# JeremyCCHsu/vae-npvc

Measured on AMD Instinct MI355X. Metric: SP frames/sec (train step: fwd+bwd+Adam), higher is better.
Workload: dtype f32 tensors and accumulation / bf16x2 operands (16 mantissa bits) on the matrix cores

## Files before the change

vae-npvc_amd/csrc/gfx950_fbwd.h:

```cpp
#pragma once
#include "gfx950_fwgrad.h"

namespace vaenpvc {
namespace tuned {

enum { FB_D2, FB_D1, FB_E1, FB_COUNT };
constexpr int FB_DY2_PITCH = 516;
constexpr bool fb_enc(int l) { return l == FB_E1; }
constexpr int fb_gsite(int l) { return l == FB_D2 ? CV_D2G : l == FB_D1 ? CV_D1G : CV_E1G; }
constexpr int fb_wsite(int l) { return l == FB_D2 ? CW_D2 : l == FB_D1 ? CW_D1 : CW_E1; }
constexpr int fb_cgr(int l) { return l == FB_D2 ? 1 : l == FB_D1 ? 2 : 4; }
#ifndef VAENPVC_FB_PFW
#define VAENPVC_FB_PFW 0x330
#endif
constexpr int fb_pfw(int l) { return (VAENPVC_FB_PFW >> (4 * l)) & 0xf; }

#ifndef VAENPVC_FB_OTL
#define VAENPVC_FB_OTL 1
#endif
#ifndef VAENPVC_FB_ABL
#define VAENPVC_FB_ABL 0
#endif
#ifndef VAENPVC_FB_XROT
#define VAENPVC_FB_XROT 0x313
// ... 7 lines not shown
  static constexpr CvSite V = CVS[fb_gsite(L)];
  static constexpr CwSite WS = CWS[fb_wsite(L)];
  static constexpr ClDesc GD = CLD[ENC ? WS.a : WS.b], XD = CLD[ENC ? WS.b : WS.a];
  static constexpr int CG = GD.C, HG = GD.H, NG = CG * HG, CX = XD.C, HX = XD.H;
  static constexpr int R = WS.R, R16 = rup(R, 16), TAPS = WS.T, S = 3;
  static constexpr int CPLG = (CG == 32 || CG == 64 || CG == 128) ? CG + 8 : CG;
  static constexpr int CPLX = (CX == 32 || CX == 64 || CX == 128) ? CX + 8 : CX;
  static constexpr int VIEWROWS = S * (R16 - 1) + TAPS + 1;
  static constexpr int ROW0G = GD.HLO, ROWSG = ENC ? fb_max(GD.HP, GD.HLO + R16) : VIEWROWS;
  static constexpr int ROW0X = ENC ? XD.HLO : 0, ROWSX = ENC ? VIEWROWS : R16;
  static constexpr int GPL = ROWSG * CPLG + 64, XPL = ROWSX * CPLX + 64;
  static constexpr int KS = cdiv(V.NT * CG, 16), MT = cdiv(V.M, 32), WP = V.Kp + 8, WPL = MT * 32 * WP;
  static constexpr int RSTEP = (V.step / CG) * CPLG;
  static constexpr int CVW = ENC ? CX : CG, CPLV = ENC ? CPLX : CPLG, CPN = ENC ? CG : CX, CPLN = ENC ? CPLG : CPLX;
  static constexpr int N = TAPS * CVW, M = WS.M, NT = cdiv(N, 32), MTW = cdiv(M, 32);
  static constexpr int KSPLIT = NT <= 2 ? 2 : 1, WN = 4 / KSPLIT, NTW = cdiv(NT, WN);
  static constexpr int CGR = fb_cgr(L), CUG = CG / CGR, NCHG = cdiv(HG, 64), NITG = NCHG * CGR, IPWG = cdiv(NITG, 4);
  static constexpr bool OTL = VAENPVC_FB_OTL != 0;
  static constexpr bool LNB2_OK = OTL && L == FB_D1 && NPL <= 2;
  static constexpr ClDesc PD0 = CLD[CL_GD0];
  static constexpr int P0_CPL = PD0.CP + 8, P0_IMG = PD0.HP * P0_CPL;
  static constexpr int OFR = CX * HX, LDS_IMG = NPL * (GPL + XPL + WPL) * 2, LDS = LDS_IMG + (OTL ? OFR * 4 : 0);
  static constexpr int LDS_LNB2 = LDS + OFR * 4 + 2 * NPL * P0_IMG * 2;
  static_assert(!OTL || (LDS_IMG % 16 == 0 && OFR % 4 == 0), "result tile: aligned, whole pieces");
  static_assert(V.x == (ENC ? WS.a : WS.b) && GD.CP == CG && XD.CP == CX && M == CPN && CUG == 8 && 4 % CGR == 0, "layer not served");
  static_assert(V.OC == CX && V.OH == HX && V.PH == (ENC ? 1 : 0) && (ENC || (V.R == R && MT == 1)), "layer not served");
  static_assert(KS * 16 <= V.Kp && (V.R - 1) * RSTEP + (KS * 16 / CG + 1) * CPLG <= ROWSG * CPLG + 64, "view runs past the frame image");
};

struct FbArgs {
  const float* dy;
  const float* a;
  const float* st;
  const float* gamma;
  const float* beta;
  const float* xa;
  const float* xst;
  const float* xgamma;
  const float* xbeta;
  const unsigned short* W;
  float* dx;
  float* dW;
  float* dgamma;
  float* dbeta;
  float* dbias;
  int F;
  bool bf16_act = false;
  int dy_pitch = 0;
  unsigned short* pl0 = nullptr;
  int64_t pl0_plane = 0;
  float* part0 = nullptr;
};

#ifndef VAENPVC_FB_OCC3
#define VAENPVC_FB_OCC3 0
#endif
#ifndef VAENPVC_FB_MAXPL
#define VAENPVC_FB_MAXPL 3
#endif
constexpr int fb_occ(int l, bool lnb2) { return (!lnb2 && ((VAENPVC_FB_OCC3 >> l) & 1)) ? 3 : 2; }
template <int NPL, int L, int BFM = 0, int DYP = 0, bool LNB2 = false>
__global__ void __launch_bounds__(256, fb_occ(L, LNB2)) k_fbwd(FbArgs a) {
  using T = FbCfg<NPL, L>;
  static_assert(!LNB2 || (T::LNB2_OK && BFM == 0), "LayerNorm backward of the layer below: decoder layer 1, fp32 storage");
  constexpr bool BFG = BFM & 1, BFX = (BFM >> 1) & 1, BFO = (BFM >> 2) & 1;
  constexpr int PG = act_pitch(BFG, T::HG), PO = act_pitch(BFO, T::V.OH), PD = DYP ? DYP : PG;
  static_assert(DYP == 0 || (BFM == 0 && DYP >= T::HG), "padded rows: fp32 storage");
  static_assert(BFM == 0 || (NPL == 1 && !T::ENC), "bf16 storage: decoder layers of the bf16 mode");
  constexpr CvSite V = T::V;
  constexpr int CUG = T::CUG, HG = T::HG, CGR = T::CGR, NITG = T::NITG, IPWG = T::IPWG;
  extern __shared__ __attribute__((aligned(16))) unsigned short bsm[];
  __shared__ float part[2][FbCfg<NPL, L>::NITG];
  __shared__ float red[4][3 * FbCfg<NPL, L>::CUG];
  __shared__ float lnx[2][FbCfg<NPL, L>::CX];
  __shared__ float red0[2][4][2];
  __shared__ float lnq0[2][LNB2 ? FbCfg<NPL, L>::CX : 1];
  float* xh0 = reinterpret_cast<float*>(reinterpret_cast<unsigned char*>(bsm) + T::LDS);
  unsigned short* img0 = reinterpret_cast<unsigned short*>(xh0 + T::OFR);
  unsigned short* gs = bsm;
  unsigned short* xs = bsm + NPL * T::GPL;
  unsigned short* ws = xs + NPL * T::XPL;
  const int tid = threadIdx.x, lane = tid & 63, wave = __builtin_amdgcn_readfirstlane(tid >> 6), l31 = lane & 31, lh = lane >> 5;
  const int cg = wave % CGR;
  const int xwave = (wave + T::XROT) & 3;
  float gam[CUG], bet[CUG];
#pragma unroll
  for (int c = 0; c < CUG; ++c) {
    gam[c] = __builtin_bit_cast(float, __builtin_amdgcn_readfirstlane(__builtin_bit_cast(int, a.gamma[cg * CUG + c])));
    bet[c] = __builtin_bit_cast(float, __builtin_amdgcn_readfirstlane(__builtin_bit_cast(int, a.beta[cg * CUG + c])));
  }
  float vd[IPWG][CUG], va[IPWG][CUG], mean = 0.f, rstd = 1.f;
  FwStage<NPL, T::CX, T::CX, T::CPLX, T::HX, 1, 0, T::ROW0X, T::XPL, BFX> sx;
  float su[CUG], sw[CUG], sd[CUG];
#pragma unroll
  for (int c = 0; c < CUG; ++c) su[c] = sw[c] = sd[c] = 0.f;

  auto uload = [&](int f, auto which_) __attribute__((always_inline)) {
    constexpr int WHICH = decltype(which_)::value;
    if constexpr ((WHICH & 2) != 0) {
      mean = a.st[2 * f];
      rstd = a.st[2 * f + 1];
// ... 84 lines not shown
    const u32x4 z = {0u, 0u, 0u, 0u};
    for (int i = tid; i < NPL * (T::GPL + T::XPL) / 8; i += 256) reinterpret_cast<u32x4*>(bsm)[i] = z;
    constexpr int WROW8 = V.Kp / 8, WPIECES = NPL * T::MT * 32 * WROW8;
    for (int i = tid; i < WPIECES; i += 256) {
      const int p = i / (T::MT * 32 * WROW8), r = i - p * (T::MT * 32 * WROW8), m = r / WROW8, c8 = r - m * WROW8;
      *reinterpret_cast<u32x4*>(ws + p * T::WPL + m * T::WP + c8 * 8) =
          *reinterpret_cast<const u32x4*>(a.W + ((size_t)p * V.Mp + m) * V.Kp + c8 * 8);
    }
  }
  const int c0 = tid >> 3, t8 = tid & 7;
  float g0 = 0.f, b0 = 0.f, su0 = 0.f, sw0 = 0.f, sd0 = 0.f;
  if constexpr (LNB2) {
    g0 = a.xgamma[c0];
    b0 = a.xbeta[c0];
    const u32x4 z = {0u, 0u, 0u, 0u};
    for (int i = tid; i < 2 * NPL * T::P0_IMG / 8; i += 256) reinterpret_cast<u32x4*>(img0)[i] = z;
    if (blockIdx.x == 0) {
      const int64_t used = (int64_t)a.F * T::PD0.HP * T::PD0.CP;
      for (int64_t i = used + tid; i < a.pl0_plane; i += 256)
#pragma unroll
        for (int p = 0; p < NPL; ++p) a.pl0[p * a.pl0_plane + i] = 0;
    }
  }
  auto copy_out0 = [&](int fp, int par) __attribute__((always_inline)) {
    constexpr int G8 = T::PD0.CP / 8, PPP = T::PD0.HP * G8;
    const unsigned short* im = img0 + par * NPL * T::P0_IMG;
    unsigned short* df = a.pl0 + (int64_t)fp * T::PD0.HP * T::PD0.CP;
#pragma unroll
    for (int r = 0; r < cdiv(NPL * PPP, 256); ++r) {
      const int it = min(tid + 256 * r, NPL * PPP - 1);
      const int p = it / PPP, q = it - p * PPP, hp = q / G8, g8 = q - hp * G8;
      const u32x4 v = *reinterpret_cast<const u32x4*>(im + p * T::P0_IMG + hp * T::P0_CPL + 8 * g8);
      *reinterpret_cast<u32x4*>(df + p * a.pl0_plane + (int64_t)q * 8) = v;
    }
  };
  int nfr = 0;
  int fprev = -1;
  __syncthreads();
  const int wn = wave % T::WN, kpar = wave / T::WN;
  f32x16 wacc[T::NTW][T::MTW];
#pragma unroll
  for (int i = 0; i < T::NTW; ++i)
#pragma unroll
    for (int j = 0; j < T::MTW; ++j) wacc[i][j] = zero16();
  const int trow = ((lane & 15) >> 2) + 8 * lh, tcol = 4 * (lane & 3) + 16 * ((lane >> 4) & 1);
  int vcol[T::NTW], pcol[T::MTW];
#pragma unroll
  for (int i = 0; i < T::NTW; ++i) {
    int n = 32 * (wn + i * T::WN) + tcol;
    n = n < T::N ? n : 0;
    vcol[i] = (n / T::CVW) * T::CPLV + n % T::CVW;
  }
#pragma unroll
  for (int j = 0; j < T::MTW; ++j) {
    const int m = 32 * j + tcol;
    pcol[j] = m < T::CPN ? m : 0;
  }
  const unsigned short* vimg = T::ENC ? xs : gs;
  const unsigned short* pimg = T::ENC ? gs + T::ROW0G * T::CPLG : xs;
  constexpr int VPL = T::ENC ? T::XPL : T::GPL, PPL = T::ENC ? T::GPL : T::XPL;
  const int woff = l31 * T::WP + lh * 8;
  for (; f < a.F; f += gridDim.x) {
    if (T::PFW != 3) {
      if constexpr (T::PFW != 3) uload(f, WTOP{});
      sx.load(a.xa, a.xst, f, a.F, xwave, lane);
    }
    upass1();
    sx.store(xs, true, lnx[0], lnx[1], xwave, lane, LNB2 ? xh0 : nullptr);
    __syncthreads();
    upass2();
    __syncthreads();
    if (T::PFW && f + (int)gridDim.x < a.F) {
      uload(f + gridDim.x, WPF{});
      if (T::PFW == 3) sx.load(a.xa, a.xst, f + gridDim.x, a.F, xwave, lane);
    }
    constexpr int NSTEPS = cdiv(V.R, 32);
    for (int s = (T::KSPLIT > 1 ? 3 - wave : wave); s < ((VAENPVC_FB_ABL & 1) ? 0 : NSTEPS); s += 4) {
      int q = s * 32 + l31;
      const bool nok = q < V.R;
      q = nok ? q : 0;
      const int xoff = q * T::RSTEP;
      f32x16 acc[T::MT];
#pragma unroll
      for (int i = 0; i < T::MT; ++i) acc[i] = zero16();
#pragma unroll
      for (int ks = 0; ks < T::KS; ++ks) {
        u32x4 fa[T::MT][NPL], fb[NPL];
        const int ko = fc_koff<T::CG, T::CPLG>(ks, lh);
#pragma unroll
        for (int p = 0; p < NPL; ++p) {
#pragma unroll
          for (int i = 0; i < T::MT; ++i) fa[i][p] = *reinterpret_cast<const u32x4*>(ws + p * T::WPL + i * 32 * T::WP + woff + ks * 16);
          fb[p] = *reinterpret_cast<const u32x4*>(gs + p * T::GPL + xoff + ko);
        }
        using PR = Prod<NPL>;
#pragma unroll
        for (int t = 0; t < PR::N; ++t)
// ... 105 lines not shown
        red0[par][wave][1] = s2;
      }
      __syncthreads();
      constexpr float INVN0 = 1.0f / T::OFR;
      s1 = ((red0[par][0][0] + red0[par][1][0]) + (red0[par][2][0] + red0[par][3][0])) * INVN0;
      s2 = ((red0[par][0][1] + red0[par][1][1]) + (red0[par][2][1] + red0[par][3][1])) * INVN0;
      if (fprev >= 0) copy_out0(fprev, par ^ 1);
      unsigned short* im = img0 + par * NPL * T::P0_IMG;
#pragma unroll
      for (int j = 0; j < EPT0; ++j) {
        const int h = t8 + 8 * j;
        if (h >= HX) continue;
        const float d = rstd0 * (dn[j] * g0 - s1 - xh[j] * s2);
        su0 += dn[j] * xh[j];
        sw0 += dn[j];
        sd0 += d;
        unsigned t[NPL];
        split_n<NPL>(d, t);
#pragma unroll
        for (int p = 0; p < NPL; ++p) im[p * T::P0_IMG + (T::PD0.HLO + h) * T::P0_CPL + c0] = (unsigned short)t[p];
      }
      fprev = f;
      ++nfr;
    } else if constexpr (T::OTL && BFM == 0) {
      if (!((VAENPVC_FB_ABL & (1 | 4)) && a.F > 0)) {
        const f32x4* ot4 = reinterpret_cast<const f32x4*>(reinterpret_cast<const unsigned char*>(bsm) + T::LDS_IMG);
        f32x4* og = reinterpret_cast<f32x4*>(a.dx + (int64_t)f * T::OFR);
        constexpr int N4 = T::OFR / 4;
#pragma unroll
        for (int r = 0; r < cdiv(N4, 256); ++r) {
          const int i = min(tid + 256 * r, N4 - 1);
          og[i] = ot4[i];
        }
      }
    }
  }
  if constexpr (LNB2) {
    __syncthreads();
    if (fprev >= 0) copy_out0(fprev, (nfr - 1) & 1);
#pragma unroll
    for (int o = 1; o < 8; o <<= 1) {
      su0 += __shfl_xor(su0, o);
      sw0 += __shfl_xor(sw0, o);
      sd0 += __shfl_xor(sd0, o);
    }
    if (t8 == 0) {
      float* pp = a.part0 + (int64_t)blockIdx.x * (3 * T::CX);
      pp[c0] = su0;
      pp[T::CX + c0] = sw0;
      pp[2 * T::CX + c0] = sd0;
    }
  }
  if ((VAENPVC_FB_ABL & 16) && a.F > 0) return;
#pragma unroll
  for (int i = 0; i < T::NTW; ++i)
#pragma unroll
    for (int j = 0; j < T::MTW; ++j) {
      const int m = 32 * j + l31;
      if (m >= T::M) continue;
#pragma unroll
      for (int reg = 0; reg < 16; ++reg) {
        const int n = 32 * (wn + i * T::WN) + acc_row(reg, lane);
        if (n < T::N && wn + i * T::WN < T::NT) atomicAdd(a.dW + n * T::M + m, wacc[i][j][reg]);
      }
    }
#pragma unroll
  for (int c = 0; c < CUG; ++c) {
    const float u = wave_sum(su[c]), w = wave_sum(sw[c]), d = wave_sum(sd[c]);
    if (lane == 0) {
      red[wave][c] = u;
      red[wave][CUG + c] = w;
      red[wave][2 * CUG + c] = d;
    }
  }
  __syncthreads();
  if (tid < 3 * T::CG) {
    const int which = tid / T::CG, c = tid - which * T::CG, cgi = c / CUG, cc = c - cgi * CUG;
    float v = 0.f;
#pragma unroll
    for (int w4 = 0; w4 < 4; ++w4)
      if (w4 % CGR == cgi) v += red[w4][which * CUG + cc];
    float* dst = which == 0 ? a.dgamma + c : which == 1 ? a.dbeta + c : a.dbias + c;
    atomicAdd(dst, v);
  }
}

template <int NPL, int L>
static unsigned fbwd_grid(int64_t F) {
  using T = FbCfg<NPL, L>;
  return (unsigned)cmin_((int)F, T::LDS > 78 * 1024 ? 256 : (fb_occ(L, false) == 3 && 3 * T::LDS <= 156 * 1024) ? 768 : 512);
}
static unsigned fbwd_grid_d1(int npl, int64_t F) { return npl == 1 ? fbwd_grid<1, FB_D1>(F) : fbwd_grid<2, FB_D1>(F); }

template <int NPL, int L>
static void launch_fbwd(const FbArgs& a, hipStream_t s) {
  using T = FbCfg<NPL, L>;
  const unsigned grid = fbwd_grid<NPL, L>(a.F);
  if constexpr (NPL == 1 && (L == FB_D2 || L == FB_D1)) {
    if (a.bf16_act) {
      constexpr int BFM = L == FB_D2 ? 7 : 1;
      rt().ensure_lds(reinterpret_cast<const void*>(&k_fbwd<NPL, L, BFM>), T::LDS);
      hipLaunchKernelGGL((k_fbwd<NPL, L, BFM>), dim3(grid), dim3(256), T::LDS, s, a);
      return;
    }
  }
  if constexpr (T::LNB2_OK) {
    if (a.pl0) {
      rt().ensure_lds(reinterpret_cast<const void*>(&k_fbwd<NPL, L, 0, 0, true>), T::LDS_LNB2);
      hipLaunchKernelGGL((k_fbwd<NPL, L, 0, 0, true>), dim3(grid), dim3(256), T::LDS_LNB2, s, a);
      return;
    }
  }
  if constexpr (L == FB_D2) {
    if (a.dy_pitch == FB_DY2_PITCH) {
      rt().ensure_lds(reinterpret_cast<const void*>(&k_fbwd<NPL, L, 0, FB_DY2_PITCH>), T::LDS);
      hipLaunchKernelGGL((k_fbwd<NPL, L, 0, FB_DY2_PITCH>), dim3(grid), dim3(256), T::LDS, s, a);
      return;
    }
  }
  rt().ensure_lds(reinterpret_cast<const void*>(&k_fbwd<NPL, L>), T::LDS);
  hipLaunchKernelGGL((k_fbwd<NPL, L>), dim3(grid), dim3(256), T::LDS, s, a);
}
template <int NPL>
static bool fbwd(int layer, const FbArgs& a, hipStream_t s) {
  if constexpr (NPL <= VAENPVC_FB_MAXPL) {
    switch (layer) {
      case FB_D2: launch_fbwd<NPL, FB_D2>(a, s); return true;
      case FB_D1: launch_fbwd<NPL, FB_D1>(a, s); return true;
      case FB_E1: launch_fbwd<NPL, FB_E1>(a, s); return true;
    }
  }
  return false;
}

}
// ... 2 lines not shown
```

vae-npvc_amd/csrc/gfx950_layers.hip:

```cpp
#include <cstdlib>
#include <cstring>
#include <type_traits>

#include "gfx950_convgemm.h"
#include "gfx950_convwgrad.h"
#include "gfx950_dense.h"
#include "gfx950_elem.h"
#include "gfx950_tngemm.h"
#include "gfx950_toeplitz.h"
#include "gfx950_toep_bf16.h"
#include "gfx950_planegemm.h"
#include "gfx950_ntring.h"
#include "gfx950_viewconv.h"
#include "gfx950_fconv.h"
#include "gfx950_fwgrad.h"
#include "gfx950_fconv_r.h"
#include "gfx950_fbwd.h"
#include "gfx950_lnb_planes.h"
#include "kernels.h"

namespace vaenpvc {
namespace tuned {

#ifndef E1F_T
// ... 120 lines not shown
  static constexpr int gd2 = d2f + D2F::BTOTAL;
  static constexpr int gd0 = gd2 + GD2::BTOTAL;
  static constexpr int ge4 = gd0 + GD0::BTOTAL;
  static constexpr int ge3 = ge4 + GE4::BTOTAL;
  static constexpr int ge2 = ge3 + GE3::BTOTAL;
  static constexpr int ge1 = ge2 + GE2::BTOTAL;
  static constexpr int wc = ge1 + GE1::BTOTAL;
  static constexpr int lnpart = wc + TOEP_C * WROW;
  static constexpr int wdg = lnpart + 2048 * 3 * 256;
  static constexpr int wfw = wdg + TB_WFLOATS;
  static constexpr int heads_bias = wfw + TB_WFLOATS;
  static constexpr int pg_headsf = heads_bias + 256;
  static constexpr int pg_headsb = pg_headsf + 3 * 256 * 768 / 2;
  static constexpr int pg_mergef = pg_headsb + 3 * 768 * 256 / 2;
  static constexpr int pg_mergeb = pg_mergef + 3 * 1664 * 128 / 2;
  static constexpr int pg_enc4f = pg_mergeb + 3 * 128 * 1600 / 2;
  static constexpr int pg_enc4b = pg_enc4f + 3 * 768 * 896 / 2;
  static constexpr int pg_bias4 = pg_enc4b + 3 * 896 * 768 / 2;
  static constexpr int cvw = pg_bias4 + 768;
  static constexpr int cvwr_d0f = cvw + CV_WTOTAL;
  static constexpr int cvwr_e2g = cvwr_d0f + fcr_wfloats(CV_D0F);
  static constexpr int enc0part_ = cvwr_e2g + fcr_wfloats(CV_E2G);
  static constexpr int enc0part = enc0part_;
  static constexpr int total = enc0part + 512 * 7 * 16;
};
static_assert(Pk::total <= 8 * 939162 + 65536, "packed weights must fit the scratch region");
static inline bool sel(unsigned mask, int bit) { return (mask >> bit) & 1u; }
static inline bool fwd_on(int bit) { return sel(rt().fwd_mask, bit); }
static inline bool bwd_on(int bit) { return sel(rt().bwd_mask, bit); }
constexpr unsigned SEL_STEPS = (2u << VAENPVC_SEL_DEC3) - 1;
constexpr int64_t PLANEGEMM_MIN_FRAMES = 1024;
static inline bool pg_on(unsigned mask, int64_t F) {
  return sel(mask, VAENPVC_SEL_PLANE_GEMM) && (F >= PLANEGEMM_MIN_FRAMES || !sel(mask, VAENPVC_SEL_PLANE_GEMM_MIN_FRAMES));
}
static inline bool pg_fwd(int64_t F) { return pg_on(rt().fwd_mask, F); }
static inline bool cg_fwd(int64_t F) { return fwd_on(VAENPVC_SEL_VIEW_GEMM) && pg_on(rt().fwd_mask | (1u << VAENPVC_SEL_PLANE_GEMM), F); }
static inline bool cg_bwd(int64_t F) { return bwd_on(VAENPVC_SEL_VIEW_GEMM) && pg_on(rt().bwd_mask | (1u << VAENPVC_SEL_PLANE_GEMM), F); }
static inline bool pg_bwd(int64_t F) { return pg_on(rt().bwd_mask, F); }
static inline bool pg_step(int bit, int64_t F) { return bwd_on(bit) && pg_bwd(F) && pg_fwd(F) && fwd_on(bit); }
static inline bool cv_sel(unsigned mask, int site) { return !sel(mask, VAENPVC_SEL_CV_SITE_SET) || ((rt().cv_sites() >> site) & 1u); }
static inline bool cv_fwd(int site, int64_t F) { return cg_fwd(F) && cv_sel(rt().fwd_mask, site); }
static inline bool cv_bwd(int site, int64_t F) { return cg_bwd(F) && cv_sel(rt().bwd_mask, site); }
constexpr int64_t FCONV_MIN_FRAMES = 1024;
constexpr int64_t ENC0_WAVE_MIN_FRAMES = 1024;
static inline bool enc0_wave(unsigned mask, int64_t F) { return F >= ENC0_WAVE_MIN_FRAMES || !sel(mask, VAENPVC_SEL_ENC0_WAVE_MIN_FRAMES); }
static inline bool fc_on(unsigned mask, int site, int64_t F) {
  if (!fconv_serves(site, rt().planes)) return false;
// ... 646 lines not shown
  else if (toep_planes)
    for_planes([&](auto npl) {
      constexpr int NPL_ = decltype(npl)::value;
      auto launch_dp = [&](auto kern) {
        VAENPVC_TIMED("dxh_post", s, hipLaunchKernelGGL(kern, dim3((unsigned)cmin_(2048, cdiv((int)F, 4))), dim3(256), 0, s, w.d_xh, P + m.dec[3].w_off,
                           reinterpret_cast<unsigned short*>(w.toep_gp), w.dy_tmp, G + m.dec[3].b_off, (int)F, dy2_pitch(F)));
      };
      if constexpr (NPL_ == 1) {
        if (abf) { launch_dp(k_dxh_post<1, true>); return; }
      }
      launch_dp(k_dxh_post<NPL_, false>);
    });
  ready();
  bool dec_bias_done[4] = {false, false, false, false};
  bool enc_bias_done[5] = {false, false, false, false, false};
  const int WGS = 512;
  const int LWGS = 2048;
  LnReduceList lnq_store;
  lnq_store.n = 0;
  lnq_store.used = 0;
  lnq_store.capacity = (int64_t)2048 * 3 * 256;
  LnReduceList* lnq = (F <= 512 && (rt().bwd_mask & SEL_STEPS) == SEL_STEPS) ? &lnq_store : nullptr;
  const bool enc0_fused = bwd_on(VAENPVC_SEL_ENC0) && bwd_on(VAENPVC_SEL_ENC1) && bwd_on(VAENPVC_SEL_ENC0_FUSED_BWD) && F >= ENC0_WAVE_MIN_FRAMES && !lnq;

  auto gsplit = [&](int cl, const float* src, const char* tag) {
    for_planes([&](auto npl) {
      VAENPVC_TIMED(tag, s, cv_split<decltype(npl)::value>(cl, src, nullptr, nullptr, nullptr, w.cl[cl], F, s));
    });
  };
  auto asplit = [&](int cl, const float* src, const float* st, const ConvL* ln, const char* tag) {
    for_planes([&](auto npl) {
      VAENPVC_TIMED(tag, s, cv_split<decltype(npl)::value>(cl, src, st, ln ? P + ln->gamma_off : nullptr, ln ? P + ln->beta_off : nullptr,
                                                           w.cl[cl], F, s));
    });
  };
  auto vwgrad = [&](int wsite, float* dW, const char* tag) {
    for_planes([&](auto npl) {
      VAENPVC_TIMED(tag, s2, cv_wgrad<decltype(npl)::value>(wsite, w.cl[CWS[wsite].a], w.cl[CWS[wsite].b], dW, F, 512, s2));
    });
  };
  auto fdgrad = [&](int site, const float* grad, float* out, const char* tag) {
    for_planes([&](auto npl) {
      FcArgs fa{grad, nullptr, nullptr, nullptr, nullptr, reinterpret_cast<const unsigned short*>(w.scratch + Pk::cvw + cv_woff(site)), nullptr, out, F};
      VAENPVC_TIMED(tag, s, fconv<decltype(npl)::value>(site, fa, s));
    });
  };
// ... 84 lines not shown
                                                            w.dy_tmp, (int)F, ToepLna{}));
        };
        if constexpr (NPL == 1) {
          if (abf) { launch_dg(&k_toep_gemm_bf16<false, 1, true>); return; }
        }
        if (dy2_pitch(F) == DY2_PITCH) launch_dg(&k_toep_gemm_bf16<false, NPL, false, DY2_PITCH>);
        else launch_dg(&k_toep_gemm_bf16<false, NPL, false>);
      });
    } else
    if (F >= 8192) {
      VAENPVC_TIMED("dec3_dgrad", s, hipLaunchKernelGGL((k_toep_dgrad<8, 8>), dim3((unsigned)cdiv(F, 32), 1), dim3(512), TD_LDS, s, w.d_xh,
                                                        w.scratch + Pk::wc, w.dy_tmp, F));
    } else {
      VAENPVC_TIMED("dec3_dgrad", s, hipLaunchKernelGGL((k_toep_dgrad<1, 4>), dim3((unsigned)cdiv(F, 32), 8), dim3(256), TD_LDS, s, w.d_xh,
                                                        w.scratch + Pk::wc, w.dy_tmp, F));
    }
    if (!(bwd_on(VAENPVC_SEL_DEC2) && fb_bwd(FB_D2, F))) {
      VAENPVC_TIMED("lnb_dec2", s, launch_ln_bwd<LnbCfg<8, 513>>(w.dy_tmp, w.dec_a[2], w.dec_st[2], P + l2.gamma_off, P + l2.beta_off, w.d_dec_a[2],
                                       G + l2.gamma_off, G + l2.beta_off, G + l2.b_off, w.scratch + Pk::lnpart, F, LWGS, s, lnq));
      dec_bias_done[2] = true;
    }
  } else generic::bwd_dec_layer(m, P, F, w, G, s, 3);
  auto fused_bwd = [&](int layer, int i, const float* dy, float* dx, const char* tag, unsigned short* pl0 = nullptr, int64_t pl0_plane = 0,
                       float* part0 = nullptr) {
    const bool enc = fb_enc(layer);
    const ConvL &l = enc ? m.enc[i] : m.dec[i], &pl = enc ? m.enc[i - 1] : m.dec[i - 1];
    float* const* act = enc ? w.enc_a : w.dec_a;
    float* const* sts = enc ? w.enc_st : w.dec_st;
    for_planes([&](auto npl) {
      constexpr int NPL = decltype(npl)::value;
      FbArgs fa{dy, act[i], sts[i], P + l.gamma_off, P + l.beta_off, act[i - 1], sts[i - 1], P + pl.gamma_off,
                P + pl.beta_off, reinterpret_cast<const unsigned short*>(w.scratch + Pk::cvw + cv_woff(fb_gsite(layer))), dx,
                G + l.w_off, G + l.gamma_off, G + l.beta_off, G + l.b_off, F};
      fa.bf16_act = abf && !enc;
      fa.dy_pitch = (layer == FB_D2 && dy2_pitch(F) == DY2_PITCH) ? DY2_PITCH : 0;
      fa.pl0 = pl0;
      fa.pl0_plane = pl0_plane;
      fa.part0 = part0;
      VAENPVC_TIMED(tag, s, fbwd<NPL>(layer, fa, s));
    });
  };
  const float* dy_cur = w.dy_tmp;

  if (bwd_on(VAENPVC_SEL_DEC2) && bwd_on(VAENPVC_SEL_DEC3) && fb_bwd(FB_D2, F)) {
    const ConvL& pl = m.dec[1];
    fused_bwd(FB_D2, 2, w.dy_tmp, w.d_dec_a[2], "dec2_bwd");
    dy_cur = w.d_dec_a[2];
    if (!(bwd_on(VAENPVC_SEL_DEC1) && fb_bwd(FB_D1, F))) {
      VAENPVC_TIMED("lnb_dec1", s, launch_ln_bwd<LnbCfg<16, 171>>(dy_cur, w.dec_a[1], w.dec_st[1], P + pl.gamma_off, P + pl.beta_off, w.d_dec_a[1],
                                        G + pl.gamma_off, G + pl.beta_off, G + pl.b_off, w.scratch + Pk::lnpart, F, LWGS, s, lnq));
      dec_bias_done[1] = true;
    }
  } else if (bwd_on(VAENPVC_SEL_DEC2)) {
    const ConvL &l = m.dec[2], &pl = m.dec[1];
    WgArgs a{w.d_dec_a[2], nullptr, nullptr, nullptr, w.dec_a[1], w.dec_st[1], P + pl.gamma_off, P + pl.beta_off,
             G + l.w_off, F, 0};
    const bool fg = fc_bwd(CV_D2G, F), vg = !fg && cv_bwd(CV_D2G, F), fw = fw_bwd(CW_D2, F), vw = !fw && cw_bwd(CW_D2, F);
    if (vg || vw) gsplit(CL_GD2, w.d_dec_a[2], "dec2_gsplit");
    if (vw && !fwd_planes(VAENPVC_SEL_DEC2, CV_D2F, F)) asplit(CL_YD1, w.dec_a[1], w.dec_st[1], &pl, "dec2_asplit");
    ready();
    if (fw) fwg(CW_D2, w.dec_a[1], w.dec_st[1], &pl, w.d_dec_a[2], nullptr, nullptr, G + l.w_off, "dec2_wgrad");
// ... 293 lines not shown
    if (vg || vw) gsplit(CL_GE2, w.d_enc_a[2], "enc2_gsplit");
    if (vw && !fwd_planes(VAENPVC_SEL_ENC2, CV_E2F, F)) asplit(CL_Y1, w.enc_a[1], w.enc_st[1], &pl, "enc2_asplit");
    ready();
    if (fw) fwg(CW_E2, w.d_enc_a[2], nullptr, nullptr, w.enc_a[1], w.enc_st[1], &pl, G + l.w_off, "enc2_wgrad");
    else if (vw) vwgrad(CW_E2, G + l.w_off, "enc2_wgrad");
    else VAENPVC_TIMED("enc2_wgrad", s2, launch_convwgrad<WE2>(wg_enc(2), WGS, s2));
    if (!enc_bias_done[2]) generic::bias_grad(w.d_enc_a[2], G + l.b_off, F, l.cout, l.hout, s);
    if (rg) rdgrad(CV_E2G, w.scratch + Pk::cvwr_e2g, w.d_enc_a[2], w.dy_tmp, "enc2_dgrad");
    else if (fg) fdgrad(CV_E2G, w.d_enc_a[2], w.dy_tmp, "enc2_dgrad");
    else if (vg) vdgrad(CV_E2G, w.dy_tmp, "enc2_dgrad");
    else
    VAENPVC_TIMED("enc2_dgrad", s, (F < SMALL_BATCH_FRAMES ? launch_convgemm<GE2s>(conv_args(w.d_enc_a[2], nullptr, nullptr, nullptr, w.scratch + Pk::ge2,
                                                                  nullptr, w.dy_tmp, F), nsplit_for<GE2s>(F), s) : launch_convgemm<GE2>(conv_args(w.d_enc_a[2], nullptr, nullptr, nullptr, w.scratch + Pk::ge2,
                                                                  nullptr, w.dy_tmp, F), nsplit_for<GE2>(F), s)));
    if (!(bwd_on(VAENPVC_SEL_ENC1) && fb_bwd(FB_E1, F))) {
      VAENPVC_TIMED("lnb_enc1", s, launch_ln_bwd<LnbCfg<32, 57>>(w.dy_tmp, w.enc_a[1], w.enc_st[1], P + pl.gamma_off, P + pl.beta_off, w.d_enc_a[1],
                                       G + pl.gamma_off, G + pl.beta_off, G + pl.b_off, w.scratch + Pk::lnpart, F, LWGS, s, lnq));
      enc_bias_done[1] = true;
    }
  } else generic::bwd_enc_layer(m, P, x, F, w, G, s, 2);
  const float* dy_e0 = w.dy_tmp;
  if (bwd_on(VAENPVC_SEL_ENC1) && bwd_on(VAENPVC_SEL_ENC2) && fb_bwd(FB_E1, F)) {
    const ConvL& pl = m.enc[0];
    fused_bwd(FB_E1, 1, w.dy_tmp, w.d_enc_a[0], "enc1_bwd");
    dy_e0 = w.d_enc_a[0];
    if (!enc0_fused)
      VAENPVC_TIMED("lnb_enc0", s, launch_ln_bwd<LnbCfg<16, 171>>(dy_e0, w.enc_a[0], w.enc_st[0], P + pl.gamma_off, P + pl.beta_off, w.d_enc_a[0],
                                        G + pl.gamma_off, G + pl.beta_off, G + pl.b_off, w.scratch + Pk::lnpart, F, LWGS, s, lnq));
    enc_bias_done[0] = true;
  } else if (bwd_on(VAENPVC_SEL_ENC1)) {
    const ConvL &l = m.enc[1], &pl = m.enc[0];
    const bool fg = fc_bwd(CV_E1G, F), vg = !fg && cv_bwd(CV_E1G, F), fw = fw_bwd(CW_E1, F), vw = !fw && cw_bwd(CW_E1, F);
    if (vg || vw) gsplit(CL_GE1, w.d_enc_a[1], "enc1_gsplit");
    if (vw && !fwd_planes(VAENPVC_SEL_ENC1, CV_E1F, F)) asplit(CL_Y0, w.enc_a[0], w.enc_st[0], &pl, "enc1_asplit");
    ready();
    if (fw) fwg(CW_E1, w.d_enc_a[1], nullptr, nullptr, w.enc_a[0], w.enc_st[0], &pl, G + l.w_off, "enc1_wgrad");
    else if (vw) vwgrad(CW_E1, G + l.w_off, "enc1_wgrad");
    else VAENPVC_TIMED("enc1_wgrad", s2, launch_convwgrad<WE1>(wg_enc(1), WGS, s2));
    if (!enc_bias_done[1]) generic::bias_grad(w.d_enc_a[1], G + l.b_off, F, l.cout, l.hout, s);
    if (fg) fdgrad(CV_E1G, w.d_enc_a[1], w.dy_tmp, "enc1_dgrad");
    else if (vg) vdgrad(CV_E1G, w.dy_tmp, "enc1_dgrad");
    else
    VAENPVC_TIMED("enc1_dgrad", s, launch_convgemm<GE1>(conv_args(w.d_enc_a[1], nullptr, nullptr, nullptr, w.scratch + Pk::ge1,
                                                                  nullptr, w.dy_tmp, F), nsplit_for<GE1>(F), s));
    if (!enc0_fused)
    VAENPVC_TIMED("lnb_enc0", s, launch_ln_bwd<LnbCfg<16, 171>>(w.dy_tmp, w.enc_a[0], w.enc_st[0], P + pl.gamma_off, P + pl.beta_off, w.d_enc_a[0],
                                      G + pl.gamma_off, G + pl.beta_off, G + pl.b_off, w.scratch + Pk::lnpart, F, LWGS, s, lnq));
    enc_bias_done[0] = true;
  } else generic::bwd_enc_layer(m, P, x, F, w, G, s, 1);
  if (enc0_fused) {
    const ConvL& l = m.enc[0];
    const int nwg = cmin_(cdiv(F, 64), 512);
    float* pw = w.scratch + Pk::enc0part;
    float* pc = w.scratch + Pk::lnpart;
    rt().ensure_lds(reinterpret_cast<const void*>(&k_enc0_bwd_wave), Enc0BwdCfg::LDS_BYTES);
    VAENPVC_TIMED("enc0_bwd", s, hipLaunchKernelGGL(k_enc0_bwd_wave, dim3((unsigned)nwg), dim3(256), Enc0BwdCfg::LDS_BYTES, s, x, dy_e0,
                                                    w.enc_st[0], P + l.w_off, P + l.b_off, P + l.gamma_off, P + l.beta_off, pw, pc, F));
    VAENPVC_TIMED("enc0_reduce", s, hipLaunchKernelGGL(k_colsum_part, dim3(7 * 16), dim3(256), 0, s, pw, nwg, 7 * 16, G + l.w_off));
    VAENPVC_TIMED("enc0_reduce", s, hipLaunchKernelGGL(k_ln_bwd_reduce, dim3(3 * 16), dim3(256), 0, s, pc, nwg, 16, G + l.gamma_off, G + l.beta_off, G + l.b_off));
  } else if (bwd_on(VAENPVC_SEL_ENC0)) {
    const ConvL& l = m.enc[0];
    WgArgs a{x, nullptr, nullptr, nullptr, w.d_enc_a[0], nullptr, nullptr, nullptr, G + l.w_off, F, 0};
    ready();
    if (enc0_wave(rt().bwd_mask, F)) {
      const int nwg = cmin_(cdiv(F, 128), 256);
      VAENPVC_TIMED("enc0_wgrad", s2, hipLaunchKernelGGL(k_enc0_wgrad_wave, dim3((unsigned)nwg), dim3(256), 0, s2, x, w.d_enc_a[0],
                                                        w.scratch + Pk::enc0part, F));
      VAENPVC_TIMED("enc0_reduce", s2, hipLaunchKernelGGL(k_colsum_part, dim3(7 * 16), dim3(256), 0, s2, w.scratch + Pk::enc0part, nwg, 7 * 16, G + l.w_off));
    } else
    VAENPVC_TIMED("enc0_wgrad", s2, launch_convwgrad<WE0>(a, WGS, s2));
    if (!enc_bias_done[0]) generic::bias_grad(w.d_enc_a[0], G + l.b_off, F, l.cout, l.hout, s);
  } else generic::bwd_enc_layer(m, P, x, F, w, G, s, 0);
  if (lnq) flush_ln_reduce(*lnq, s);
// ... 109 lines not shown
```

vae-npvc_amd/csrc/runtime.h:

```cpp
#pragma once
#include <hip/hip_runtime.h>

#include <cstdint>
#include <cstring>
#include <string>
#include <unordered_set>
#include <utility>
#include <vector>

namespace vaenpvc {

struct Runtime {
  unsigned fwd_mask = 0xffffffffu, bwd_mask = 0xffffffffu;
  int planes = 2;
  unsigned cv_sites() const { return planes == 1 ? 0xe2ceu : planes == 2 ? 0xc244u : 0x4u; }
  static constexpr unsigned FC_SITES = 0xdb1u;
  static constexpr unsigned FCR_SITES = 0x28au;
  static constexpr unsigned FW_SITES = 0x3fu;
  long fb_layers_env = -1;
  unsigned fb_layers() const { return fb_layers_env >= 0 ? (unsigned)fb_layers_env : 0x7u; }
  bool act_bf16 = false;
  int nt_ar = 0;
  int nt_ring = 1;
  int cg_sf_ring = 1;
  int cg_pf_ring = 0;
  bool dxh_skip = true;
  bool d0g_planes = true;
  int d2_lna = 1;
  bool d2_tail = false;
  bool toep_f32 = false;
  bool side_enabled = true;
  bool side_forced = false;
  int frame_max = 512;
  int64_t last_F = -1;
  int last_path = -1, last_planes = 0;
  unsigned last_fwd_mask = 0, last_bwd_mask = 0;
  const void* last_ws = nullptr;
  int64_t plz_F = -1;
  int64_t dxh_post_F = -1;
  int device = -1;
  hipStream_t s2 = nullptr;
  hipEvent_t ev[16] = {};
  int ev_next = 0;
// ... 35 lines not shown
```

vae-npvc_amd/csrc/runtime.hip:

```cpp
#include "runtime.h"

#include <cstdlib>
#include <cstring>

namespace vaenpvc {

static thread_local Runtime* tl_rt = nullptr;
static Runtime g_detached;

Runtime& rt() { return tl_rt ? *tl_rt : g_detached; }
RtScope::RtScope(Runtime* r) : prev(tl_rt) { tl_rt = r; }
RtScope::~RtScope() { tl_rt = prev; }

void Runtime::read_env() {
  if (const char* e = getenv("VAENPVC_FWD_MASK")) fwd_mask = (unsigned)strtoul(e, nullptr, 0);
  if (const char* e = getenv("VAENPVC_BWD_MASK")) bwd_mask = (unsigned)strtoul(e, nullptr, 0);
  if (const char* e = getenv("VAENPVC_SIDE_STREAM")) {
    side_enabled = e[0] != '0';
    side_forced = side_enabled;
  }
  if (const char* e = getenv("VAENPVC_TOEP")) toep_f32 = !strcmp(e, "f32");
  if (const char* e = getenv("VAENPVC_D2_TAIL")) d2_tail = atoi(e) != 0;
  if (const char* e = getenv("VAENPVC_D2_LNA")) d2_lna = atoi(e);
  if (const char* e = getenv("VAENPVC_D0G_PLANES")) d0g_planes = atoi(e) != 0;
  if (const char* e = getenv("VAENPVC_DXH_SKIP")) dxh_skip = atoi(e) != 0;
  if (const char* e = getenv("VAENPVC_NT_RING")) nt_ring = atoi(e);
  if (const char* e = getenv("VAENPVC_CG_SF_RING")) cg_sf_ring = atoi(e);
  if (const char* e = getenv("VAENPVC_CG_PF_RING")) cg_pf_ring = atoi(e);
  if (const char* e = getenv("VAENPVC_NT_AR")) nt_ar = atoi(e);
  if (const char* e = getenv("VAENPVC_FRAME_MAX")) frame_max = atoi(e) < 0 ? 0 : (atoi(e) > 1024 ? 1024 : atoi(e));
  if (const char* e = getenv("VAENPVC_FB_LAYERS")) fb_layers_env = (long)strtoul(e, nullptr, 0);
  if (const char* e = getenv("VAENPVC_ACT_BF16")) act_bf16 = atoi(e) != 0;
  if (const char* e = getenv("VAENPVC_PLANES")) {
    int p = atoi(e);
    if (p >= 1 && p <= 3) planes = p;
  }
}

void Runtime::release() {
  if (s2) {
    (void)hipStreamSynchronize(s2);
    (void)hipStreamDestroy(s2);
    for (auto& e : ev)
      if (e) (void)hipEventDestroy(e);
  }
  s2 = nullptr;
  for (auto& e : ev) e = nullptr;
  ev_next = 0;
  for (auto& p : pool) {
    (void)hipEventDestroy(p.first);
    (void)hipEventDestroy(p.second);
  }
  pool.clear();
  used = 0;
// ... 60 lines not shown
```

Measured before the change: 5.714 million.

## Fuse encoder layer-0 backward (LayerNorm+conv weight grad) into encoder layer-1 fused backward

Adds an E0B variant of the fused backward kernel for encoder layer 1. Once dx of layer 1 is in LDS, this variant recomputes layer 0's conv output from the raw input, normalizes and applies LeakyReLU, runs the LayerNorm backward, and accumulates per-workgroup partial sums for the layer-0 weight, gamma, beta and bias gradients. Two small reduction kernels then finish those gradients. This removes the separate enc0 LayerNorm backward and enc0 weight-gradient passes along with their round trips through global memory, at the cost of extra LDS, an extra barrier and per-frame recompute inside the layer-1 kernel.

```diff
diff --git a/vae-npvc_amd/csrc/gfx950_fbwd.h b/vae-npvc_amd/csrc/gfx950_fbwd.h
--- a/vae-npvc_amd/csrc/gfx950_fbwd.h
+++ b/vae-npvc_amd/csrc/gfx950_fbwd.h
@@ -53,7 +53,12 @@
   static constexpr int P0_CPL = PD0.CP + 8, P0_IMG = PD0.HP * P0_CPL;
   static constexpr int OFR = CX * HX, LDS_IMG = NPL * (GPL + XPL + WPL) * 2, LDS = LDS_IMG + (OTL ? OFR * 4 : 0);
   static constexpr int LDS_LNB2 = LDS + OFR * 4 + 2 * NPL * P0_IMG * 2;
+  static constexpr bool E0B_OK = OTL && L == FB_E1 && NPL <= 2;
+  static constexpr int E0_H = 513, E0_TAPS = 7, E0_PPT = 11, E0_XWIN = 3 * (E0_PPT - 1) + E0_TAPS, E0_XS = 544, E0_WS = (E0_TAPS + 1) * 16;
+  static constexpr int LDS_E0B = LDS + (E0_XS + E0_WS) * 4;
   static_assert(!OTL || (LDS_IMG % 16 == 0 && OFR % 4 == 0), "result tile: aligned, whole pieces");
+  static_assert(!E0B_OK || (CX == 16 && HX == 171 && 16 * E0_PPT >= HX && 3 * (16 * E0_PPT - 1) + E0_TAPS <= E0_XS && 3 * HX == E0_H), "encoder layer 0");
+  static_assert(!E0B_OK || (LDS % 16 == 0 && LDS_E0B <= 78 * 1024), "two workgroups per CU (and the grid fbwd_grid derives from LDS)");
   static_assert(V.x == (ENC ? WS.a : WS.b) && GD.CP == CG && XD.CP == CX && M == CPN && CUG == 8 && 4 % CGR == 0, "layer not served");
   static_assert(V.OC == CX && V.OH == HX && V.PH == (ENC ? 1 : 0) && (ENC || (V.R == R && MT == 1)), "layer not served");
   static_assert(KS * 16 <= V.Kp && (V.R - 1) * RSTEP + (KS * 16 / CG + 1) * CPLG <= ROWSG * CPLG + 64, "view runs past the frame image");
@@ -81,6 +86,10 @@
   unsigned short* pl0 = nullptr;
   int64_t pl0_plane = 0;
   float* part0 = nullptr;
+  const float* x0 = nullptr;
+  const float* w0 = nullptr;
+  const float* b0 = nullptr;
+  float* part0w = nullptr;
 };
 
 #ifndef VAENPVC_FB_OCC3
@@ -90,10 +99,11 @@
 #define VAENPVC_FB_MAXPL 3
 #endif
 constexpr int fb_occ(int l, bool lnb2) { return (!lnb2 && ((VAENPVC_FB_OCC3 >> l) & 1)) ? 3 : 2; }
-template <int NPL, int L, int BFM = 0, int DYP = 0, bool LNB2 = false>
-__global__ void __launch_bounds__(256, fb_occ(L, LNB2)) k_fbwd(FbArgs a) {
+template <int NPL, int L, int BFM = 0, int DYP = 0, bool LNB2 = false, bool E0B = false>
+__global__ void __launch_bounds__(256, fb_occ(L, LNB2 || E0B)) k_fbwd(FbArgs a) {
   using T = FbCfg<NPL, L>;
   static_assert(!LNB2 || (T::LNB2_OK && BFM == 0), "LayerNorm backward of the layer below: decoder layer 1, fp32 storage");
+  static_assert(!E0B || (T::E0B_OK && BFM == 0 && !LNB2), "backward of the layer below: encoder layer 1, fp32 storage");
   constexpr bool BFG = BFM & 1, BFX = (BFM >> 1) & 1, BFO = (BFM >> 2) & 1;
   constexpr int PG = act_pitch(BFG, T::HG), PO = act_pitch(BFO, T::V.OH), PD = DYP ? DYP : PG;
   static_assert(DYP == 0 || (BFM == 0 && DYP >= T::HG), "padded rows: fp32 storage");
@@ -108,6 +118,8 @@
   __shared__ float lnq0[2][LNB2 ? FbCfg<NPL, L>::CX : 1];
   float* xh0 = reinterpret_cast<float*>(reinterpret_cast<unsigned char*>(bsm) + T::LDS);
   unsigned short* img0 = reinterpret_cast<unsigned short*>(xh0 + T::OFR);
+  float* xr0 = reinterpret_cast<float*>(reinterpret_cast<unsigned char*>(bsm) + T::LDS);
+  float* w0s = xr0 + T::E0_XS;
   unsigned short* gs = bsm;
   unsigned short* xs = bsm + NPL * T::GPL;
   unsigned short* ws = xs + NPL * T::XPL;
@@ -238,6 +250,26 @@
         for (int p = 0; p < NPL; ++p) a.pl0[p * a.pl0_plane + i] = 0;
     }
   }
+  const int c16 = tid >> 4, t16 = tid & 15;
+  float acc0[T::E0_TAPS], xq[3] = {0.f, 0.f, 0.f}, mean0q = 0.f, rstd0q = 1.f, mean0 = 0.f, rstd0 = 1.f;
+#pragma unroll
+  for (int t = 0; t < T::E0_TAPS; ++t) acc0[t] = 0.f;
+  auto xload0 = [&](int fx) __attribute__((always_inline)) {
+    const float* xf = a.x0 + (int64_t)fx * T::E0_H;
+    xq[0] = xf[tid];
+    xq[1] = xf[256 + tid];
+    xq[2] = xf[512];
+    mean0q = a.xst[2 * fx];
+    rstd0q = a.xst[2 * fx + 1];
+  };
+  if constexpr (E0B) {
+    g0 = a.xgamma[c16];
+    b0 = a.xbeta[c16];
+    for (int i = tid; i < T::E0_XS; i += 256) xr0[i] = 0.f;
+    if (tid < T::E0_TAPS * 16) w0s[tid] = a.w0[tid];
+    if (tid < 16) w0s[T::E0_TAPS * 16 + tid] = a.b0[tid];
+    if (T::PFW == 3 && f < a.F) xload0(f);
+  }
   auto copy_out0 = [&](int fp, int par) __attribute__((always_inline)) {
     constexpr int G8 = T::PD0.CP / 8, PPP = T::PD0.HP * G8;
     const unsigned short* im = img0 + par * NPL * T::P0_IMG;
@@ -280,15 +312,24 @@
     if (T::PFW != 3) {
       if constexpr (T::PFW != 3) uload(f, WTOP{});
       sx.load(a.xa, a.xst, f, a.F, xwave, lane);
+      if constexpr (E0B) xload0(f);
     }
     upass1();
     sx.store(xs, true, lnx[0], lnx[1], xwave, lane, LNB2 ? xh0 : nullptr);
     __syncthreads();
+    if constexpr (E0B) {
+      xr0[2 + tid] = xq[0];
+      xr0[2 + 256 + tid] = xq[1];
+      if (tid == 0) xr0[2 + 512] = xq[2];
+      mean0 = mean0q;
+      rstd0 = rstd0q;
+    }
     upass2();
     __syncthreads();
     if (T::PFW && f + (int)gridDim.x < a.F) {
       uload(f + gridDim.x, WPF{});
       if (T::PFW == 3) sx.load(a.xa, a.xst, f + gridDim.x, a.F, xwave, lane);
+      if constexpr (E0B && T::PFW == 3) xload0(f + gridDim.x);
     }
     constexpr int NSTEPS = cdiv(V.R, 32);
     for (int s = (T::KSPLIT > 1 ? 3 - wave : wave); s < ((VAENPVC_FB_ABL & 1) ? 0 : NSTEPS); s += 4) {
@@ -440,6 +481,51 @@
       }
       fprev = f;
       ++nfr;
+    } else if constexpr (E0B) {
+      const float* ot = reinterpret_cast<const float*>(reinterpret_cast<const unsigned char*>(bsm) + T::LDS_IMG);
+      constexpr int HX = T::HX, PPT = T::E0_PPT, TAPS = T::E0_TAPS;
+      const float* xp = xr0 + 3 * PPT * t16;
+      float wl[TAPS], dn[PPT], xh[PPT];
+      const float bl = w0s[TAPS * 16 + c16];
+#pragma unroll
+      for (int t = 0; t < TAPS; ++t) wl[t] = w0s[t * 16 + c16];
+      float s1 = 0.f, s2 = 0.f;
+#pragma unroll
+      for (int k = 0; k < PPT; ++k) {
+        const int j = PPT * t16 + k;
+        const bool ok = j < HX;
+        float a0 = bl;
+#pragma unroll
+        for (int t = 0; t < TAPS; ++t) a0 = __builtin_fmaf(wl[t], xp[3 * k + t], a0);
+        xh[k] = ok ? (a0 - mean0) * rstd0 : 0.f;
+        const float nn = __builtin_fmaf(xh[k], g0, b0);
+        dn[k] = ok ? ot[c16 * HX + (ok ? j : 0)] * (nn >= 0.f ? 1.0f : LEAK) : 0.f;
+        const float dxv = dn[k] * g0;
+        s1 += dxv;
+        s2 += dxv * xh[k];
+      }
+      s1 = wave_sum(s1);
+      s2 = wave_sum(s2);
+      const int par = nfr & 1;
+      if (lane == 0) {
+        red0[par][wave][0] = s1;
+        red0[par][wave][1] = s2;
+      }
+      __syncthreads();
+      constexpr float INVN0 = 1.0f / T::OFR;
+      s1 = ((red0[par][0][0] + red0[par][1][0]) + (red0[par][2][0] + red0[par][3][0])) * INVN0;
+      s2 = ((red0[par][0][1] + red0[par][1][1]) + (red0[par][2][1] + red0[par][3][1])) * INVN0;
+#pragma unroll
+      for (int k = 0; k < PPT; ++k) {
+        const bool ok = PPT * t16 + k < HX;
+        const float d = ok ? rstd0 * (dn[k] * g0 - s1 - xh[k] * s2) : 0.f;
+        su0 += dn[k] * xh[k];
+        sw0 += dn[k];
+        sd0 += d;
+#pragma unroll
+        for (int t = 0; t < TAPS; ++t) acc0[t] += xp[3 * k + t] * d;
+      }
+      ++nfr;
     } else if constexpr (T::OTL && BFM == 0) {
       if (!((VAENPVC_FB_ABL & (1 | 4)) && a.F > 0)) {
         const f32x4* ot4 = reinterpret_cast<const f32x4*>(reinterpret_cast<const unsigned char*>(bsm) + T::LDS_IMG);
@@ -467,6 +553,25 @@
       pp[c0] = su0;
       pp[T::CX + c0] = sw0;
       pp[2 * T::CX + c0] = sd0;
+    }
+  }
+  if constexpr (E0B) {
+#pragma unroll
+    for (int o = 1; o < 16; o <<= 1) {
+#pragma unroll
+      for (int t = 0; t < T::E0_TAPS; ++t) acc0[t] += __shfl_xor(acc0[t], o);
+      su0 += __shfl_xor(su0, o);
+      sw0 += __shfl_xor(sw0, o);
+      sd0 += __shfl_xor(sd0, o);
+    }
+    if (t16 == 0) {
+      float* pw = a.part0w + (int64_t)blockIdx.x * (T::E0_TAPS * 16);
+#pragma unroll
+      for (int t = 0; t < T::E0_TAPS; ++t) pw[t * 16 + c16] = acc0[t];
+      float* pp = a.part0 + (int64_t)blockIdx.x * (3 * T::CX);
+      pp[c16] = su0;
+      pp[T::CX + c16] = sw0;
+      pp[2 * T::CX + c16] = sd0;
     }
   }
   if ((VAENPVC_FB_ABL & 16) && a.F > 0) return;
@@ -504,11 +609,16 @@
 }
 
 template <int NPL, int L>
+constexpr int fbwd_grid_max() {
+  using T = FbCfg<NPL, L>;
+  return T::LDS > 78 * 1024 ? 256 : (fb_occ(L, false) == 3 && 3 * T::LDS <= 156 * 1024) ? 768 : 512;
+}
+template <int NPL, int L>
 static unsigned fbwd_grid(int64_t F) {
-  using T = FbCfg<NPL, L>;
-  return (unsigned)cmin_((int)F, T::LDS > 78 * 1024 ? 256 : (fb_occ(L, false) == 3 && 3 * T::LDS <= 156 * 1024) ? 768 : 512);
+  return (unsigned)cmin_((int)F, fbwd_grid_max<NPL, L>());
 }
 static unsigned fbwd_grid_d1(int npl, int64_t F) { return npl == 1 ? fbwd_grid<1, FB_D1>(F) : fbwd_grid<2, FB_D1>(F); }
+static unsigned fbwd_grid_e1(int npl, int64_t F) { return npl == 1 ? fbwd_grid<1, FB_E1>(F) : fbwd_grid<2, FB_E1>(F); }
 
 template <int NPL, int L>
 static void launch_fbwd(const FbArgs& a, hipStream_t s) {
@@ -529,6 +639,13 @@
       return;
     }
   }
+  if constexpr (T::E0B_OK) {
+    if (a.x0) {
+      rt().ensure_lds(reinterpret_cast<const void*>(&k_fbwd<NPL, L, 0, 0, false, true>), T::LDS_E0B);
+      hipLaunchKernelGGL((k_fbwd<NPL, L, 0, 0, false, true>), dim3(grid), dim3(256), T::LDS_E0B, s, a);
+      return;
+    }
+  }
   if constexpr (L == FB_D2) {
     if (a.dy_pitch == FB_DY2_PITCH) {
       rt().ensure_lds(reinterpret_cast<const void*>(&k_fbwd<NPL, L, 0, FB_DY2_PITCH>), T::LDS);
diff --git a/vae-npvc_amd/csrc/gfx950_layers.hip b/vae-npvc_amd/csrc/gfx950_layers.hip
--- a/vae-npvc_amd/csrc/gfx950_layers.hip
+++ b/vae-npvc_amd/csrc/gfx950_layers.hip
@@ -166,7 +166,8 @@
   static constexpr int cvwr_e2g = cvwr_d0f + fcr_wfloats(CV_D0F);
   static constexpr int enc0part_ = cvwr_e2g + fcr_wfloats(CV_E2G);
   static constexpr int enc0part = enc0part_;
-  static constexpr int total = enc0part + 512 * 7 * 16;
+  static constexpr int enc0cpart = enc0part + 512 * 7 * 16;
+  static constexpr int total = enc0cpart + 512 * 3 * 16;
 };
 static_assert(Pk::total <= 8 * 939162 + 65536, "packed weights must fit the scratch region");
 static inline bool sel(unsigned mask, int bit) { return (mask >> bit) & 1u; }
@@ -859,6 +860,8 @@
   lnq_store.capacity = (int64_t)2048 * 3 * 256;
   LnReduceList* lnq = (F <= 512 && (rt().bwd_mask & SEL_STEPS) == SEL_STEPS) ? &lnq_store : nullptr;
   const bool enc0_fused = bwd_on(VAENPVC_SEL_ENC0) && bwd_on(VAENPVC_SEL_ENC1) && bwd_on(VAENPVC_SEL_ENC0_FUSED_BWD) && F >= ENC0_WAVE_MIN_FRAMES && !lnq;
+  const bool enc0_in_enc1 = rt().fb_enc0 && rt().planes <= 2 && bwd_on(VAENPVC_SEL_ENC0) && bwd_on(VAENPVC_SEL_ENC1) && bwd_on(VAENPVC_SEL_ENC2) &&
+                            fb_bwd(FB_E1, F);
 
   auto gsplit = [&](int cl, const float* src, const char* tag) {
     for_planes([&](auto npl) {
@@ -989,7 +992,7 @@
     }
   } else generic::bwd_dec_layer(m, P, F, w, G, s, 3);
   auto fused_bwd = [&](int layer, int i, const float* dy, float* dx, const char* tag, unsigned short* pl0 = nullptr, int64_t pl0_plane = 0,
-                       float* part0 = nullptr) {
+                       float* part0 = nullptr, const float* x0 = nullptr, float* part0w = nullptr) {
     const bool enc = fb_enc(layer);
     const ConvL &l = enc ? m.enc[i] : m.dec[i], &pl = enc ? m.enc[i - 1] : m.dec[i - 1];
     float* const* act = enc ? w.enc_a : w.dec_a;
@@ -1004,6 +1007,12 @@
       fa.pl0 = pl0;
       fa.pl0_plane = pl0_plane;
       fa.part0 = part0;
+      if (x0) {
+        fa.x0 = x0;
+        fa.w0 = P + pl.w_off;
+        fa.b0 = P + pl.b_off;
+        fa.part0w = part0w;
+      }
       VAENPVC_TIMED(tag, s, fbwd<NPL>(layer, fa, s));
     });
   };
@@ -1343,9 +1352,18 @@
   const float* dy_e0 = w.dy_tmp;
   if (bwd_on(VAENPVC_SEL_ENC1) && bwd_on(VAENPVC_SEL_ENC2) && fb_bwd(FB_E1, F)) {
     const ConvL& pl = m.enc[0];
-    fused_bwd(FB_E1, 1, w.dy_tmp, w.d_enc_a[0], "enc1_bwd");
+    if (enc0_in_enc1) {
+      static_assert(FbCfg<1, FB_E1>::E0B_OK && FbCfg<2, FB_E1>::E0B_OK, "the form enc0_in_enc1 selects");
+      const int nwg = (int)fbwd_grid_e1(rt().planes, F);
+      float* pw = w.scratch + Pk::enc0part;
+      float* pc = w.scratch + Pk::enc0cpart;
+      static_assert(fbwd_grid_max<1, FB_E1>() <= 512 && fbwd_grid_max<2, FB_E1>() <= 512, "rows of Pk::enc0part / Pk::enc0cpart");
+      fused_bwd(FB_E1, 1, w.dy_tmp, w.d_enc_a[0], "enc1_bwd", nullptr, 0, pc, x, pw);
+      VAENPVC_TIMED("enc0_reduce", s, hipLaunchKernelGGL(k_colsum_part, dim3(7 * 16), dim3(256), 0, s, pw, nwg, 7 * 16, G + pl.w_off));
+      VAENPVC_TIMED("enc0_reduce", s, hipLaunchKernelGGL(k_ln_bwd_reduce, dim3(3 * 16), dim3(256), 0, s, pc, nwg, 16, G + pl.gamma_off, G + pl.beta_off, G + pl.b_off));
+    } else fused_bwd(FB_E1, 1, w.dy_tmp, w.d_enc_a[0], "enc1_bwd");
     dy_e0 = w.d_enc_a[0];
-    if (!enc0_fused)
+    if (!enc0_fused && !enc0_in_enc1)
       VAENPVC_TIMED("lnb_enc0", s, launch_ln_bwd<LnbCfg<16, 171>>(dy_e0, w.enc_a[0], w.enc_st[0], P + pl.gamma_off, P + pl.beta_off, w.d_enc_a[0],
                                         G + pl.gamma_off, G + pl.beta_off, G + pl.b_off, w.scratch + Pk::lnpart, F, LWGS, s, lnq));
     enc_bias_done[0] = true;
@@ -1369,7 +1387,8 @@
                                       G + pl.gamma_off, G + pl.beta_off, G + pl.b_off, w.scratch + Pk::lnpart, F, LWGS, s, lnq));
     enc_bias_done[0] = true;
   } else generic::bwd_enc_layer(m, P, x, F, w, G, s, 1);
-  if (enc0_fused) {
+  if (enc0_in_enc1) {
+  } else if (enc0_fused) {
     const ConvL& l = m.enc[0];
     const int nwg = cmin_(cdiv(F, 64), 512);
     float* pw = w.scratch + Pk::enc0part;
diff --git a/vae-npvc_amd/csrc/runtime.h b/vae-npvc_amd/csrc/runtime.h
--- a/vae-npvc_amd/csrc/runtime.h
+++ b/vae-npvc_amd/csrc/runtime.h
@@ -19,6 +19,7 @@
   static constexpr unsigned FW_SITES = 0x3fu;
   long fb_layers_env = -1;
   unsigned fb_layers() const { return fb_layers_env >= 0 ? (unsigned)fb_layers_env : 0x7u; }
+  bool fb_enc0 = true;
   bool act_bf16 = false;
   int nt_ar = 0;
   int nt_ring = 1;
diff --git a/vae-npvc_amd/csrc/runtime.hip b/vae-npvc_amd/csrc/runtime.hip
--- a/vae-npvc_amd/csrc/runtime.hip
+++ b/vae-npvc_amd/csrc/runtime.hip
@@ -30,6 +30,7 @@
   if (const char* e = getenv("VAENPVC_NT_AR")) nt_ar = atoi(e);
   if (const char* e = getenv("VAENPVC_FRAME_MAX")) frame_max = atoi(e) < 0 ? 0 : (atoi(e) > 1024 ? 1024 : atoi(e));
   if (const char* e = getenv("VAENPVC_FB_LAYERS")) fb_layers_env = (long)strtoul(e, nullptr, 0);
+  if (const char* e = getenv("VAENPVC_FB_ENC0")) fb_enc0 = atoi(e) != 0;
   if (const char* e = getenv("VAENPVC_ACT_BF16")) act_bf16 = atoi(e) != 0;
   if (const char* e = getenv("VAENPVC_PLANES")) {
     int p = atoi(e);
```

Result: no change. 5.739 million (median of 6 runs) (+0.5%).
